# leodd/Lifted-Hybrid-Variational-Inference

Measured on AMD Instinct MI355X. Metric: lbp_sweeps_per_sec_10M_edge_hybrid_mrf, higher is better.
Workload: dtype f64

## Files before the change

### include/lhvi.h

```cpp
#ifndef LHVI_H
#define LHVI_H

#include <stddef.h>
#include <stdint.h>

#ifdef __cplusplus
extern "C" {
#endif

#define LHVI_ABI_VERSION 21
#define LHVI_MAX_ARITY 6

#define LHVI_OK 0
#define LHVI_E_ARG (-1)
#define LHVI_E_LAUNCH (-2)
#define LHVI_E_UNSUPPORTED (-3)
#define LHVI_E_NODEVICE (-4)
#define LHVI_E_NOT_PD (-5)

#define LHVI_POT_GENERIC 0
#define LHVI_POT_TABLE 1
#define LHVI_POT_GAUSSIAN 2
#define LHVI_POT_QUADRATIC 3
#define LHVI_POT_HYBRID_QUADRATIC 4
#define LHVI_POT_LINEAR_GAUSSIAN 5
#define LHVI_POT_X2 6
#define LHVI_POT_XY 7
#define LHVI_POT_MLN 8
#define LHVI_POT_MLN_HARD 9
#define LHVI_POT_IMAGE_NODE 10
#define LHVI_POT_IMAGE_EDGE 11

typedef struct lhvi_graph {
// ... 168 lines not shown
int lhvi_pbp_classify(const lhvi_graph_t* g, const lhvi_pots_t* pots, const lhvi_pbp_t* s, uint8_t* edge_class, void* stream);

int lhvi_pbp_uniq(const lhvi_graph_t* g, int32_t n, const double* particles, const int32_t* np, uint8_t* uniq, void* stream);
int lhvi_pbp_v2f(const lhvi_graph_t* g, const lhvi_pbp_t* s, const double* f2v, double* v2f, void* stream);
int lhvi_pbp_f2v(const lhvi_graph_t* g, const lhvi_pots_t* pots, const lhvi_pbp_t* s, const double* v2f, double* f2v, void* stream);
int lhvi_pbp_proposal(const lhvi_graph_t* g, const lhvi_pbp_t* s, const double* f2v, double* eta, double* q, void* stream);
int lhvi_pbp_proposal_partial(const lhvi_graph_t* g, const lhvi_pbp_t* s, const double* f2v, double* eta, double* ph, void* stream);
int lhvi_pbp_proposal_finish(const lhvi_graph_t* g, const lhvi_pbp_t* s, const double* ph, double* q, void* stream);
int lhvi_pbp_boundary_pack(const lhvi_graph_t* g, const lhvi_pbp_t* s, const double* f2v, const double* ph, int32_t nb,
                           const int32_t* bvars, double* send, void* stream);
int lhvi_pbp_boundary_reduce(int32_t n_items, const int32_t* width, const int32_t* src_ptr, const int64_t* src_off,
                             const int32_t* dst_ptr, const int64_t* dst_off, const double* in, double* out, void* stream);
int lhvi_pbp_init(const lhvi_graph_t* g, const lhvi_pbp_t* s, double* eta, double* q, double* f2v, double* v2f, void* stream);
int lhvi_pbp_resample(const lhvi_graph_t* g, const lhvi_pbp_t* s, const int64_t* var_gid, uint64_t seed, uint32_t iteration, double* particles_out, void* stream);
int lhvi_pbp_edge_points(const lhvi_graph_t* g, const lhvi_pots_t* pots, const lhvi_pbp_t* s, const double* v2f,
                         int32_t nq, const int32_t* qedge, int32_t npts, const double* x, double* out, void* stream);
int lhvi_pbp_resample_uniq(const lhvi_graph_t* g, const lhvi_pbp_t* s, const int64_t* var_gid, uint64_t seed, uint32_t iteration,
                           double* particles_out, uint8_t* uniq_out, void* stream);
int lhvi_pbp_belief_points(const lhvi_graph_t* g, const lhvi_pots_t* pots, const lhvi_pbp_t* s, const double* v2f,
                           int32_t nq, const int32_t* qvar, int32_t npts, const double* x, double* out, void* stream);
int lhvi_pbp_var_fused(const lhvi_graph_t* g, const lhvi_pbp_t* s, const double* f2v, double* v2f, double* eta, double* q,
                       const int64_t* var_gid, uint64_t seed, uint32_t iteration, double* particles_out, uint8_t* uniq_out,
                       const int32_t* desc, int32_t n16, int32_t n32_t32, int32_t n32_t64, void* stream);
int lhvi_pbp_quad(const lhvi_graph_t* g, const lhvi_pots_t* pots, const lhvi_pbp_t* s, const double* v2f, int64_t nq,
                  const int32_t* row_var, const int64_t* qptr, const int32_t* qedge, const double* qmult, const double* lo,
                  const double* hi, double epsabs, double epsrel, double* z, double* abserr, int32_t* status, void* stream);
int lhvi_pbp_map_brent(const lhvi_graph_t* g, const lhvi_pots_t* pots, const lhvi_pbp_t* s, const double* v2f, int64_t nq,
                       const int32_t* row_var, const int64_t* qptr, const int32_t* qedge, const double* qmult, double xtol,
                       int32_t maxfun, double* xout, double* fout, int32_t* nfev, void* stream);

int lhvi_pbp_halo_pack(const double* v2f, int32_t n, int32_t n_rows, const int32_t* row_edge, const int64_t* row_off,
                       const int32_t* row_width, const double* q, int32_t n_q, const int32_t* q_var, const int64_t* q_off,
                       double* out, void* stream);
int lhvi_pbp_halo_unpack(const double* in, int32_t n, int32_t n_rows, const int32_t* row_edge, const int64_t* row_off,
                         const int32_t* row_width, double* v2f, int32_t n_q, const int32_t* q_var, const int64_t* q_off,
                         double* q, void* stream);


typedef struct lhvi_vi {
    int32_t K;
    int32_t T;
    int32_t Dmax;
    int32_t quirks;
    const double* gh_x;
    const double* gh_w;
    const double* w;
// ... 262 lines not shown
```

### lifted-hybrid-variational-inference_amd/csrc/pbp.hip

```cpp
#include "common.hpp"
#include "potential.hpp"
#include "fastmath.hpp"
#include "cq.hpp"

namespace lhvi {

__device__ __forceinline__ double wave_sum(double v) { return dpp_wave_reduce(v, SumOp()); }
__device__ __forceinline__ double wave_max(double v) { return dpp_wave_reduce(v, MaxOp()); }
__device__ __forceinline__ int wave_sum_i(int v) {
#pragma unroll
    for (int off = 32; off > 0; off >>= 1) v += __shfl_xor(v, off);
    return v;
}

constexpr double PAD_LOG_TERM = -6.0e5;

__host__ __device__ __forceinline__ int var_first(const lhvi_pbp_t& s) { return s.var_hi > s.var_lo ? s.var_lo : 0; }
__host__ __device__ __forceinline__ int var_limit(const lhvi_graph_t& g, const lhvi_pbp_t& s) { return s.var_hi > s.var_lo ? s.var_hi : g.V; }

__device__ __forceinline__ double norm_pdf_std(double x, double mu, double sig) {
    const double u = (x - mu) / sig;
    return exp(-u * u * 0.5) / (2.506628274631 * sig);
}

// ... 2434 lines not shown
                uint64_t todo = dp & live;
                dp = 0;
                while (todo) {
                    const int k = __builtin_ctzll(todo);
                    const int klo = __builtin_amdgcn_readlane(xlo[h], k), khi = __builtin_amdgcn_readlane(xhi[h], k);
                    const uint64_t same = __ballot(xlo[h] == klo && xhi[h] == khi) & live;
                    dp |= same & (same - 1);
                    todo &= ~same;
                }
            }
            const int u = (lane < cn) && !((dp >> lane) & 1);
            if (lane < n) uniq[(int64_t)vv[h] * n + lane] = (uint8_t)u;
        }
    }
}

#ifndef LHVI_FUSED_WAVES
#define LHVI_FUSED_WAVES 4
#endif
constexpr int FUSED_CH = 8;
#ifndef LHVI_FUSED_NB
#define LHVI_FUSED_NB 2
#endif
template <int W, int PW, bool EP, bool R16>
__global__ void __launch_bounds__(BLOCK) __attribute__((amdgpu_waves_per_eu(LHVI_FUSED_WAVES, 8)))
pbp_var_fused_kernel(lhvi_graph_t g, lhvi_pbp_t s, const double* __restrict__ f2v, double* __restrict__ v2f, double* __restrict__ eta,
                     double* __restrict__ q, const int64_t* __restrict__ gid, uint64_t seed, uint32_t iteration,
                     double* __restrict__ out, uint8_t* __restrict__ uniq, const int32_t* __restrict__ list, int count) {
    __shared__ LogRec sh_log[LOG_TAB_N];
    load_log_table(sh_log);
    __syncthreads();
    constexpr int G = WAVE / W, SL = W / PW;
    const int lane = threadIdx.x & 63;
    const int64_t slot = ((int64_t)blockIdx.x * (BLOCK / WAVE) + (threadIdx.x >> 6)) * G + lane / W;
    const int j = lane % W;
    const bool on = slot < count;
    const int32_t* rec = list + (R16 ? 16 : 8) * (on ? slot : 0);
    int4 ra, rb;
    int2 rc = make_int2(0, 0);
    int e_rec = 0;
    if (R16) {
        const int4* r4 = reinterpret_cast<const int4*>(rec);
        ra = r4[0]; rb = r4[1]; rc = reinterpret_cast<const int2*>(rec)[4];
        e_rec = rec[10 + min(lane % W, 5)];
    } else {
        ra = make_int4(rec[0], rec[1], rec[2], rec[3]); rb = make_int4(rec[4], rec[5], rec[6], rec[7]);
    }
    const int v = on ? ra.x : 0;
    const int deg = on ? ra.y : 0, gb = ra.z, T = on ? ra.w : 0;
    const double dlo = __hiloint2double(rb.y, rb.x), dhi = __hiloint2double(rb.w, rb.z);
    const int n = s.n, S = s.n + s.T;
    const int np = on ? (R16 ? rc.x : s.np[v]) : 0;
    const bool valid = j < np;
    const int lo = on ? (R16 ? rc.y : g.var_ptr[v]) : 0;
    const bool lifted = g.edge_count != nullptr;
    const double q0 = on ? s.q[2 * v] : 0.0, q1 = on ? s.q[2 * v + 1] : 1.0;
    int maxdeg = deg;
#pragma unroll
    for (int off = 32; off >= W; off >>= 1) maxdeg = max(maxdeg, __shfl_xor(maxdeg, off));
    constexpr int CH = FUSED_CH;
    static_assert(W >= CH && CH % SL == 0, "lane j of a group holds edge j of the chunk");
    const int first_lane = lane / W * W;
    const int nch = (maxdeg + CH - 1) / CH;
    int my_e = 0, held = -1;
    auto hold_chunk = [&](int c) {
        if (c == held) return;
        held = c;
        if (R16 && c == 0) {
            my_e = j < deg ? (j < 6 ? e_rec : (j < CH ? g.var_edge[lo + j] : 0)) : 0;
            return;
        }
        my_e = (j < CH && c * CH + j < deg) ? g.var_edge[lo + c * CH + j] : 0;
    };
    {
        double total = 0.0;
        int ee[CH];
        double mm[CH];
        auto load_rows = [&](int c) {
            hold_chunk(c);
#pragma unroll
            for (int i = 0; i < CH; ++i) ee[i] = __shfl(my_e, first_lane + i);
#pragma unroll
            for (int i = 0; i < CH; ++i) mm[i] = f2v[(int64_t)ee[i] * S + (valid ? j : 0)];
        };
        for (int c = 0; c < nch; ++c) {
            load_rows(c);
#pragma unroll
            for (int i = 0; i < CH; ++i) {
                const double m = valid ? mm[i] : 0.0;
                if (c * CH + i < deg) total += lifted ? m * g.edge_count[ee[i]] : m;
            }
        }
        double logw = 0.0;
        bool uq = false;
        if (valid) {
            const int d = g.var_dom[v];
            const double sd = sqrt_pos(q1);
            logw = log_importance(g, s, v, d, s.particles[(int64_t)v * n + j], q0, rcp_newton(sd), log_pos(2.506628274631 * sd));
            uq = s.uniq[(int64_t)v * n + j] != 0;
        }
        auto group_sum = [&](double x) { return W == 16 ? dpp_move<0x15F>(dpp_row_reduce(x, SumOp())) : dpp_half_reduce(x, SumOp(), lane); };
        auto group_max = [&](double x) { return W == 16 ? dpp_row_reduce(x, MaxOp()) : dpp_half_reduce(x, MaxOp(), lane); };
        const uint64_t mine = (W == 16 ? 0xffffull : 0xffffffffull) << (lane / W * W);
        const double rcnt = rcp_newton(fmax((double)__builtin_popcountll(__ballot(uq) & mine), 1.0));
        for (int c = 0; c < nch; ++c) {
            if (nch > 1) load_rows(c);
#pragma unroll
            for (int i = 0; i < CH; ++i) {
                const int k = c * CH + i;
                if (k >= maxdeg) break;
                const bool live = k < deg;
                const double m = (live && valid) ? mm[i] : 0.0;
                const double res = (total - m) + logw;
                const double mean = group_sum(uq ? res : 0.0) * rcnt;
                double shift = mean;
                if (__ballot(uq && (res - mean > s.max_log_value))) {
                    const double mx = group_max(uq ? res : -__builtin_huge_val());
                    if (mx - mean > s.max_log_value) shift = mx - s.max_log_value;
                }
                if (live && valid) v2f[(int64_t)ee[i] * n + j] = res - shift;
            }
        }
    }
    double total = 0.0;
    if (lifted) for (int k = 0; k < deg; ++k) total += g.edge_count[g.var_edge[lo + k]];
    else total = (double)deg;
    const double min_sig = total * s.var_threshold;
    const int sub = j / PW, tl = j % PW;
    double ps[4] = {0.0, 0.0, 0.0, 0.0}, pm[4] = {0.0, 0.0, 0.0, 0.0};
    const int t0 = min(tl, max(T - 1, 0)), t1 = min(tl + PW, max(T - 1, 0));
    const double xg0 = g.dom_val[gb + t0], xg1 = g.dom_val[gb + t1];
    constexpr int NB = LHVI_FUSED_NB;
    for (int c = 0; c < nch; ++c) {
        hold_chunk(c);
#pragma unroll
        for (int p0 = 0; p0 < CH / SL; p0 += NB) {
            if (c * CH + p0 * SL >= maxdeg) break;
            int ee[NB];
            double b0[NB], b1[NB], g0[NB], g1[NB];
#pragma unroll
            for (int i = 0; i < NB; ++i) {
                const int kc = (p0 + i) * SL + sub;
                ee[i] = __shfl(my_e, first_lane + min(kc, CH - 1));
                if (kc >= CH || c * CH + kc >= deg) ee[i] = 0;
            }
#pragma unroll
            for (int i = 0; i < NB; ++i) {
                const double* msg = f2v + (int64_t)ee[i] * S + n;
                b0[i] = eta[2 * ee[i]]; b1[i] = eta[2 * ee[i] + 1];
                g0[i] = msg[t0]; g1[i] = msg[t1];
            }
#pragma unroll
            for (int i = 0; i < NB; ++i) {
                if (p0 + i >= CH / SL || c * CH + (p0 + i) * SL >= maxdeg) break;
                const int k = c * CH + (p0 + i) * SL + sub;
                const bool live = k < deg;
                const int e = ee[i];
                const double e0 = on ? b0[i] : 0.0, e1 = on ? b1[i] : 1.0;
                const bool use_cav = EP && !(q1 >= e1);
                double c0 = 0.0, c1 = 1.0;
                if (use_cav) gdiv(q0, q1, e0, e1, c0, c1);
                const double csd = sqrt(c1);
                double z = 0.0, a = 0.0, b = 0.0;
                if (on && tl < T) {
                    double w = exp(g0[i]);
                    if (use_cav) w = w * norm_pdf_std(xg0, c0, csd);
                    z += w; a += w * xg0; b += w * (xg0 * xg0);
                }
                if (on && tl + PW < T) {
                    double w = exp(g1[i]);
                    if (use_cav) w = w * norm_pdf_std(xg1, c0, csd);
                    z += w; a += w * xg1; b += w * (xg1 * xg1);
                }
                if (PW == 16) { z = dpp_row_reduce(z, SumOp()); a = dpp_row_reduce(a, SumOp()); b = dpp_row_reduce(b, SumOp()); }
                else { z = dpp_half_reduce(z, SumOp(), lane); a = dpp_half_reduce(a, SumOp(), lane); b = dpp_half_reduce(b, SumOp(), lane); }
                const double rz = rcp_newton(z);
                double mu = a * rz;
                double sig = b * rz - mu * mu;
                if (use_cav) { const double m0 = mu, m1 = sig; gdiv(m0, m1, c0, c1, mu, sig); }
                if (0.0 < sig && sig < __builtin_huge_val()) {
                    sig = fmax(sig, min_sig);
                    if (live && tl == 0) { eta[2 * e] = mu; eta[2 * e + 1] = sig; }
                } else {
                    mu = e0; sig = e1;
                }
                if (live) {
                    const double p = rcp_newton(sig);
                    const int slot4 = k & (WAVE / PW - 1);
                    const double cnt = lifted ? g.edge_count[e] : 1.0;
#pragma unroll
                    for (int r = 0; r < 4; ++r)
                        if (r == slot4) {
                            if (lifted) { ps[r] += p * cnt; pm[r] += p * mu * cnt; }
                            else { ps[r] += p; pm[r] += p * mu; }
                        }
                }
            }
        }
    }
    double fs, fm;
    if (PW == 16 && SL == 1) { fs = (ps[0] + ps[1]) + (ps[2] + ps[3]); fm = (pm[0] + pm[1]) + (pm[2] + pm[3]); }
    else if (PW == 16) {
        const double s01 = (sub == 0 ? ps[0] : ps[1]), s23 = (sub == 0 ? ps[2] : ps[3]);
        const double m01 = (sub == 0 ? pm[0] : pm[1]), m23 = (sub == 0 ? pm[2] : pm[3]);
        fs = (s01 + __shfl_xor(s01, 16)) + (s23 + __shfl_xor(s23, 16));
        fm = (m01 + __shfl_xor(m01, 16)) + (m23 + __shfl_xor(m23, 16));
    } else { fs = ps[0] + ps[1]; fm = pm[0] + pm[1]; }
    fs = 1.0 / fs;
    const double mu_new = fs * fm, var_new = fs;
    if (on && j == 0) { q[2 * v] = mu_new; q[2 * v + 1] = var_new; }
    const double mu_b = __shfl(mu_new, first_lane), sd_b = sqrt_pos(__shfl(var_new, first_lane));
    double x = 0.0;
    if (valid) {
        double zc, zs;
        philox_normal_pair(seed, gid ? (uint64_t)gid[v] : (uint64_t)v, (uint32_t)j, iteration, sh_log, zc, zs);
        x = fmin(fmax(fma(sd_b, zc, mu_b), dlo), dhi) + 0.0;
        out[(int64_t)v * n + j] = x;
    }
    int u = valid;
    for (int k = 0; k + 1 < W; ++k) {
        const double xk = __shfl(x, first_lane + k);
        if (k < j && k < np && xk == x) u = 0;
    }
    if (on && j < n) uniq[(int64_t)v * n + j] = (uint8_t)u;
}

static int validate_pbp(const lhvi_graph_t* g, const lhvi_pbp_t* s) {
    if (!g || !s) return LHVI_E_ARG;
    if (g->V < 0 || g->E < 0 || s->n <= 0 || s->T < 0) return LHVI_E_ARG;
    if (g->V > 0 && (!g->var_ptr || !g->var_edge || !g->var_value || !g->var_dom || !g->dom_cont || !g->dom_ptr ||
                     !s->particles || !s->np)) return LHVI_E_ARG;
    if (s->var_hi > s->var_lo ? (s->var_lo < 0 || s->var_hi > g->V) : (s->var_lo != 0 || s->var_hi != 0)) return LHVI_E_ARG;
    return LHVI_OK;
}

}

using namespace lhvi;

template <bool HALO>
static int launch_v2f(const lhvi_graph_t* g, const lhvi_pbp_t* s, const double* f2v, double* v2f, void* stream) {
    if (s->v2f_wide || s->v2f_narrow) {
        if (!s->v2f_wide || !s->v2f_narrow || s->n_v2f_wide < 0 || s->n_v2f_narrow < 0 || s->bslot || s->var_hi > s->var_lo) return LHVI_E_ARG;
        if (s->n_v2f_wide > 0)
            hipLaunchKernelGGL(pbp_v2f_kernel<HALO>, dim3(grid_for((int64_t)s->n_v2f_wide * WAVE)), dim3(BLOCK), 0, as_stream(stream), *g, *s, f2v, v2f);
// ... 383 lines not shown
    hipStream_t st = as_stream(stream);
    const bool ep = (s->flags & LHVI_PBP_EP) != 0;
#define LHVI_FUSED(W, PW, list, cnt)                                                                                                  \
    if ((cnt) > 0) {                                                                                                                  \
        const dim3 grid(grid_for(((int64_t)(cnt) + WAVE / (W) - 1) / (WAVE / (W)) * WAVE));                                          \
        if (ep && r16) hipLaunchKernelGGL((pbp_var_fused_kernel<W, PW, true, true>), grid, dim3(BLOCK), 0, st, *g, *s, f2v, v2f, eta, q, var_gid, \
                                   seed, iteration, particles_out, uniq_out, list, cnt);                                             \
        else if (ep) hipLaunchKernelGGL((pbp_var_fused_kernel<W, PW, true, false>), grid, dim3(BLOCK), 0, st, *g, *s, f2v, v2f, eta, q, var_gid, \
                                   seed, iteration, particles_out, uniq_out, list, cnt);                                             \
        else if (r16) hipLaunchKernelGGL((pbp_var_fused_kernel<W, PW, false, true>), grid, dim3(BLOCK), 0, st, *g, *s, f2v, v2f, eta, q, var_gid,   \
                                seed, iteration, particles_out, uniq_out, list, cnt);                                                \
        else hipLaunchKernelGGL((pbp_var_fused_kernel<W, PW, false, false>), grid, dim3(BLOCK), 0, st, *g, *s, f2v, v2f, eta, q, var_gid,   \
                                seed, iteration, particles_out, uniq_out, list, cnt);                                                \
    }
    const bool r16 = (s->flags & LHVI_PBP_FUSED_RECORDS16) != 0;
    const int64_t rw = r16 ? 16 : 8;
    LHVI_FUSED(16, 16, desc, n16)
    LHVI_FUSED(32, 16, desc + rw * (int64_t)n16, n32_t32)
    LHVI_FUSED(32, 32, desc + rw * ((int64_t)n16 + n32_t32), n32_t64)
#undef LHVI_FUSED
    return check_launch();
}

int lhvi_pbp_quad(const lhvi_graph_t* g, const lhvi_pots_t* pots, const lhvi_pbp_t* s, const double* v2f, int64_t nq,
                  const int32_t* row_var, const int64_t* qptr, const int32_t* qedge, const double* qmult, const double* lo,
                  const double* hi, double epsabs, double epsrel, double* z, double* abserr, int32_t* status, void* stream) {
    if (int rc = validate_pbp(g, s)) return rc;
    if (!pots || !v2f || nq < 0 || !(epsabs >= 0.0) || !(epsrel >= 0.0)) return LHVI_E_ARG;
    if (nq == 0) return LHVI_OK;
    if (!row_var || !lo || !hi || !z) return LHVI_E_ARG;
    if (qptr && (!qedge || !qmult)) return LHVI_E_ARG;
    QueryRows rows{row_var, qptr, qedge, qmult};
    hipLaunchKernelGGL(pbp_quad_kernel, dim3(grid_for(nq)), dim3(BLOCK), 0, as_stream(stream), *g, *pots, *s, v2f, nq, rows, row_var,
                       lo, hi, epsabs, epsrel, z, abserr, status);
    return check_launch();
}

}
```

### lifted-hybrid-variational-inference_amd/lhvi/_abi.py

```python
from __future__ import annotations

import ctypes as C
import os

import numpy as np

_HERE = os.path.dirname(os.path.abspath(__file__))
LIB_PATH = os.environ.get('LHVI_LIB') or os.path.join(os.path.dirname(_HERE), 'csrc', 'liblhvi.so')

c_i32p = C.c_void_p
c_f64p = C.c_void_p


class LhviError(RuntimeError):
    pass


class GraphStruct(C.Structure):
    _fields_ = [
        ('V', C.c_int32), ('F', C.c_int32), ('E', C.c_int32), ('nnz', C.c_int32),
        ('fac_ptr', C.c_void_p), ('edge_var', C.c_void_p), ('edge_fac', C.c_void_p), ('edge_canon', C.c_void_p),
        ('var_ptr', C.c_void_p), ('var_edge', C.c_void_p), ('edge_count', C.c_void_p), ('fac_pot', C.c_void_p),
        ('var_value', C.c_void_p), ('var_dom', C.c_void_p), ('var_mult', C.c_void_p), ('fac_mult', C.c_void_p),
        ('D', C.c_int32),
# ... 52 lines not shown
               [(n, C.c_double) for n in ('lr', 'b1', 'b2', 'eps', 'var_min')] + [('t', C.c_int32)]


PBP_EP = 1
PBP_EPBP_DISCRETE = 2
PBP_SKIP_TERMS = 16
PBP_NO_GRID = 128
PBP_LEAVE_ROOM = 256
PBP_BOUNDARY_TOTALS = 2048
PBP_CQ = 512
PBP_NO_UNIQ = 4096
PBP_V2F_RECORDS = 8192
PBP_WIDE_PAIRS = 16384
PBP_SHARE_CUS = 32768
PBP_POW2_GROUPS = 65536
PBP_FUSED_RECORDS16 = 131072
PBP_F2V_HEAVY = 262144
PBP_F2V_SMALL = 524288
PBP_F2V_PAIR = 1048576
PBP_F2V_FAST = 2097152
PBP_F2V_CQ = 4194304
PBP_F2V_GENERIC = 8388608
PBP_F2V_ALL = PBP_F2V_HEAVY | PBP_F2V_SMALL | PBP_F2V_PAIR | PBP_F2V_FAST | PBP_F2V_CQ | PBP_F2V_GENERIC
ABI_VERSION = 21
PBP_DESC_BYTES = 128
COLOR_HASH, COLOR_SORT = 0, 1
HUB_DEGREE = 64
VI_GROUP_SLOTS, VI_GROUP_COMP, VI_TINY_NODES, VI_TINY_K, VI_TINY_PAR = 24, 48, 32, 2, 3072

class MwsStruct(C.Structure):
    _fields_ = [('T', C.c_int32), ('max_flips', C.c_int32), ('epsilon', C.c_double), ('noise_std', C.c_double),
                ('seed', C.c_uint64), ('try_id', C.c_void_p), ('disc', C.c_void_p), ('n_disc', C.c_int32),
                ('num', C.c_void_p), ('n_num', C.c_int32), ('fac_class', C.c_void_p), ('x', C.c_void_p), ('best_x', C.c_void_p),
                ('cur_score', C.c_void_p), ('best_score', C.c_void_p), ('status', C.c_void_p), ('err_flip', C.c_void_p),
                ('rec_score', C.c_void_p), ('rec_zero', C.c_void_p), ('rec_ticks', C.c_void_p)] + \
               [(n, C.c_void_p) for n in ('rp_init', 'rp_clause', 'rp_walk', 'rp_walk_k', 'rp_noise', 'rp_post', 'out_score',
                                          'out_unsat', 'out_winner', 'out_accept', 'out_val')]


class ExactStruct(C.Structure):
    _fields_ = [('Nd', C.c_int32), ('Nc', C.c_int32), ('M', C.c_int64), ('dstates', C.c_void_p), ('dstride', C.c_void_p),
                ('n_quad', C.c_int32), ('quad_ptr', C.c_void_p), ('quad_desc', C.c_void_p), ('quad_par', C.c_void_p),
                ('n_tab', C.c_int32), ('tab_ptr', C.c_void_p), ('tab_desc', C.c_void_p), ('tab_par', C.c_void_p)]


class GibbsStruct(C.Structure):
    _fields_ = [('ex', ExactStruct), ('dstate_off', C.c_void_p), ('vt_ptr', C.c_void_p), ('vt_fac', C.c_void_p),
# ... 58 lines not shown
    'lhvi_pbp_var_sum': (C.c_int, [_G, _S, _vp, _vp, _vp]),
    'lhvi_pbp_domain_grid': (C.c_int, [_G, _S, _vp, _vp]),
    'lhvi_pbp_refine_grid': (C.c_int, [_G, _S, _vp, _vp, _vp, _vp, _vp]),
    'lhvi_debug_exp': (C.c_int, [_vp, _vp, _i64, _vp]),
    'lhvi_debug_log': (C.c_int, [_vp, _vp, _i64, C.c_int32, _vp]),
    'lhvi_debug_exp_acc': (C.c_int, [_vp, _vp, _vp, _i64, _vp]),
    'lhvi_debug_exp_acc_floor': (C.c_int, [_vp, _vp, _vp, _i64, _vp]),
    'lhvi_pbp_v2f': (C.c_int, [_G, _S, _vp, _vp, _vp]),
    'lhvi_pbp_f2v': (C.c_int, [_G, _P, _S, _vp, _vp, _vp]),
    'lhvi_pbp_proposal': (C.c_int, [_G, _S, _vp, _vp, _vp, _vp]),
    'lhvi_pbp_proposal_partial': (C.c_int, [_G, _S, _vp, _vp, _vp, _vp]),
    'lhvi_pbp_proposal_finish': (C.c_int, [_G, _S, _vp, _vp, _vp]),
    'lhvi_pbp_boundary_pack': (C.c_int, [_G, _S, _vp, _vp, _i32, _vp, _vp, _vp]),
    'lhvi_pbp_boundary_reduce': (C.c_int, [_i32, _vp, _vp, _vp, _vp, _vp, _vp, _vp, _vp]),
    'lhvi_pbp_halo_pack': (C.c_int, [_vp, _i32, _i32, _vp, _vp, _vp, _vp, _i32, _vp, _vp, _vp, _vp]),
    'lhvi_pbp_halo_unpack': (C.c_int, [_vp, _i32, _i32, _vp, _vp, _vp, _vp, _i32, _vp, _vp, _vp, _vp]),
    'lhvi_pbp_init': (C.c_int, [_G, _S, _vp, _vp, _vp, _vp, _vp]),
    'lhvi_pbp_resample': (C.c_int, [_G, _S, _vp, _u64, _u32, _vp, _vp]),
    'lhvi_pbp_edge_points': (C.c_int, [_G, _P, _S, _vp, _i32, _vp, _i32, _vp, _vp, _vp]),
    'lhvi_pbp_resample_uniq': (C.c_int, [_G, _S, _vp, _u64, _u32, _vp, _vp, _vp]),
    'lhvi_pbp_belief_points': (C.c_int, [_G, _P, _S, _vp, _i32, _vp, _i32, _vp, _vp, _vp]),
    'lhvi_pbp_map_brent': (C.c_int, [_G, _P, _S, _vp, _i64, _vp, _vp, _vp, _vp, _f64, _i32, _vp, _vp, _vp, _vp]),
    'lhvi_pbp_var_fused': (C.c_int, [_G, _S, _vp, _vp, _vp, _vp, _vp, _u64, _u32, _vp, _vp, _vp, _i32, _i32, _i32, _vp]),
    'lhvi_pbp_quad': (C.c_int, [_G, _P, _S, _vp, _i64, _vp, _vp, _vp, _vp, _vp, _vp, _f64, _f64, _vp, _vp, _vp, _vp]),
    'lhvi_vi_workspace_bytes': (_sz, [_G, _VI]),
    'lhvi_vi_grad': (C.c_int, [_G, _P, _VI, _vp, _vp, _vp, _vp, _vp, _sz, _vp]),
    'lhvi_vi_adam_run': (C.c_int, [_G, _P, _VI, C.POINTER(ViOptStruct), _i32, _vp, _vp, _sz, _vp]),
    'lhvi_adam_step': (C.c_int, [_vp, _vp, _vp, _vp, _i64, _i32, _f64, _f64, _f64, _f64, _i32, _f64, _vp]),
    'lhvi_softmax_rows': (C.c_int, [_vp, _vp, _i64, _i32, _i32, _vp]),
    'lhvi_vi_map_bfgs': (C.c_int, [_G, _VI, _i64, _vp, _f64, _i32, _vp, _vp, _vp, _vp, _vp]),
    'lhvi_color_workspace_bytes': (_sz, [_G]),
    'lhvi_color_refine_factors': (C.c_int, [_G, _vp, _vp, _vp, _vp, _vp, _vp, _sz, _i32, _vp]),
    'lhvi_color_refine_rvs': (C.c_int, [_G, _vp, _vp, _vp, _vp, _vp, _sz, _i32, _vp]),
    'lhvi_color_first_members': (C.c_int, [_vp, _i32, _i32, _vp, _vp]),
    'lhvi_color_segment_sums': (C.c_int, [_vp, _vp, _i32, _vp, _vp]),
    'lhvi_mws_init': (C.c_int, [_G, _P, C.POINTER(MwsStruct), _vp]),
    'lhvi_mws_flips': (C.c_int, [_G, _P, C.POINTER(MwsStruct), _i32, _i32, _vp]),
    'lhvi_lbfgsb_host': (C.c_int, [_i32, _vp, LBFGSB_FUN, _vp, _vp, _vp, _vp, _vp]),
    'lhvi_wall_clock_khz': (C.c_int, [_vp]),
    'lhvi_exact_lds_bytes': (_sz, [_i32, _i32, _i32]),
    'lhvi_exact_configs': (C.c_int, [C.POINTER(ExactStruct), _i64, _i64, _i32, _vp, _vp, _vp, _vp, _vp, _vp]),
    'lhvi_exact_normalize': (C.c_int, [_i64, _vp, _vp, _vp, _vp, _vp]),
    'lhvi_exact_marginals': (C.c_int, [C.POINTER(ExactStruct), _i32, _vp, _vp, _vp]),
    'lhvi_exact_mix_prepare': (C.c_int, [_i32, _i64, _vp, _vp, _vp, _vp, _vp]),
    'lhvi_exact_mixture': (C.c_int, [_i32, _i64, _vp, _i32, _vp, _vp, _vp]),
    'lhvi_exact_map_polish': (C.c_int, [_i32, _i64, _vp, _i32, _vp, _vp, _vp, _vp, _i32, _vp, _vp]),
# ... 227 lines not shown
```

### lifted-hybrid-variational-inference_amd/lhvi/pbp.py

```python
from __future__ import annotations

import os
from math import e, log, sqrt

import numpy as np

from . import _abi
from .flat import flatten

_F2V_LONG = _abi.PBP_F2V_HEAVY | _abi.PBP_F2V_SMALL
_F2V_SHORT = _abi.PBP_F2V_PAIR | _abi.PBP_F2V_FAST | _abi.PBP_F2V_CQ | _abi.PBP_F2V_GENERIC
F2V_SCHEDULES = {
    'one': (('main', _abi.PBP_F2V_ALL, 0, False),),
    'timed': (('main', _F2V_LONG, 0, True), ('main', _F2V_SHORT, 0, False)),
    'overlap': (('side', _F2V_SHORT, 0, False), ('main', _F2V_LONG, _abi.PBP_SHARE_CUS, True)),
}


class _ParticleSweep:
    var_threshold = 3
    max_log_value = 700
    _epbp_discrete = True
    verbose = False
    listed_proposal = True
    dynamic_f2v = True
    paired_light = True
    cq_routing = True
    small_f2v = True
    long_grid_min_edges = 1 << 16
    listed_resample = True
    sliced_proposal = True
    prop_slice = 64
    packed_v2f = True
    overlap_f2v = True
    overlap_min_heavy = 1 << 16
    fused_var_kernel = True
    fused_max_particles = 32
    exact_queries = False
    map_mode = 'fminbound'

    def _setup(self, graph_like, flat=None, edge_key=None, sides='vf', edge_skip=None, owned=None):
        flat = flat if flat is not None else flatten(graph_like, require_device_potentials=True)
        self.flat = flat
        self.dg = dg = _abi.DeviceGraph(flat)
        torch = _abi.require_gpu()
        n = self.n
        sizes = np.diff(flat.dom_ptr)
        cont = flat.dom_cont.astype(bool)
        self.T = int(sizes[cont].max()) if cont.any() else 0
        nst = flat.var_nstates
        if (flat.var_hidden & ~flat.var_cont & (nst > n)).any():
            raise _abi.LhviError('a discrete variable has more states than particle slots n=%d' % n)
        if (flat.var_hidden & flat.var_cont & (np.diff(flat.var_ptr) == 0)).any():
            raise ZeroDivisionError('a hidden continuous variable has no incident factor: its proposal is an empty product')
        self.np_host = np.where(flat.var_hidden, np.where(flat.var_cont, n, nst), 0).astype(np.int32)
        host_lists = {'np_dev': self.np_host}
        S = n + self.T
        self.f2v = dg.zeros(flat.E, S)
        self.v2f = dg.zeros(flat.E, n)
        self.eta = dg.zeros(flat.E, 2)
# ... 47 lines not shown
            pd = np.concatenate([sl, np.delete(pd, hubs, axis=0)])
            host_lists['prop_hub'], self.n_prop_hub = ph, int(hubs.size)
            self.prop_partial = dg.zeros(owner.size, 2)
        host_lists['prop_desc'] = np.ascontiguousarray(pd) if pv.size else None
        self.n_prop_desc = int(pd.shape[0])
        hidden_v = np.flatnonzero(flat.var_hidden)
        if owned is not None:
            hidden_v = hidden_v[hidden_v < owned]
        narrow = self.np_host[hidden_v] <= 4
        self.v2f_lists = None
        hub = ~narrow & (np.diff(flat.var_ptr)[hidden_v] > 64) & (self.np_host[hidden_v] <= 64)
        mid16 = ~narrow & ~hub & (self.np_host[hidden_v] <= 16)
        mid32 = ~narrow & ~hub & ~mid16 & (self.np_host[hidden_v] <= 32)
        if self.packed_v2f and hidden_v.size and (narrow.any() or hub.any() or mid16.any() or mid32.any()):
            wide = ~narrow & ~hub & ~mid16 & ~mid32
            parts = (('wide', wide), ('narrow', narrow), ('hub', hub), ('mid16', mid16), ('mid32', mid32))
            for name, m in parts:
                host_lists['v2f_' + name] = hidden_v[m].astype(np.int32) if m.any() else np.zeros(1, dtype=np.int32)
            if os.environ.get('LHVI_PBP_V2F_REC', '1') != '0':
                host_lists['v2f_wide'] = self._v2f_records(flat, hidden_v[wide])
        self._fused = None
        pT = sizes[pdom] if pv.size else np.zeros(0, dtype=np.int64)
        fused_max = int(os.environ.get('LHVI_PBP_FUSED_MAX', self.fused_max_particles))
        fz = (pdeg <= min(64, self.prop_slice)) & (pT <= 64) & (n <= min(32, fused_max)) if pv.size else np.zeros(0, dtype=bool)
        if (self.fused_var_kernel and os.environ.get('LHVI_PBP_FUSED', '1') != '0') and owned is None and self.sampler == 'device' and self.listed_proposal and self.listed_resample \
                and 'v2f_wide' in host_lists and fz.any():
            k16 = fz & (n <= 16) & (pT <= 32)
            k32a = fz & ~k16 & (pT <= 32)
            k32b = fz & ~k16 & ~k32a
            wide_rec = os.environ.get('LHVI_PBP_FUSED_REC16', '1') != '0'
            fd = np.zeros((pv.size, 16 if wide_rec else 8), dtype=np.int32)
            fd[:, 0], fd[:, 1], fd[:, 2], fd[:, 3] = pv, pdeg, flat.dom_ptr[pdom], pT
            fd[:, 4:6] = np.ascontiguousarray(flat.dom_lo[pdom], dtype=np.float64).view(np.int32).reshape(-1, 2)
            fd[:, 6:8] = np.ascontiguousarray(flat.dom_hi[pdom], dtype=np.float64).view(np.int32).reshape(-1, 2)
            if wide_rec:
                fd[:, 8], fd[:, 9] = self.np_host[pv], flat.var_ptr[pv]
                for k in range(6):
                    has = pdeg > k
                    fd[has, 10 + k] = flat.var_edge[pbase[has] + k]
                self.flags |= _abi.PBP_FUSED_RECORDS16
            host_lists['fused_desc'] = np.ascontiguousarray(np.concatenate([fd[k16], fd[k32a], fd[k32b]]))
            fused_var = np.zeros(flat.V, dtype=bool)
            fused_var[pv[fz]] = True
            keep = ~fused_var[pd[:, 0]]
            host_lists['prop_desc_rest'] = np.ascontiguousarray(pd[keep]) if keep.any() else np.zeros((1, 8), dtype=np.int32)
            rkeep = ~fused_var[rr[:, 0]]
            host_lists['resample_rest'] = np.ascontiguousarray(rr[rkeep]) if rkeep.any() else np.zeros((1, 8), dtype=np.int32)
            rest_parts = []
            if 'v2f_wide' in host_lists:
                for name, m in parts:
                    vs = hidden_v[m]
                    vs = vs[~fused_var[vs]]
                    host_lists['v2f_rest_' + name] = (self._v2f_records(flat, vs) if name == 'wide' and os.environ.get('LHVI_PBP_V2F_REC', '1') != '0' else
                                                      vs.astype(np.int32) if vs.size else np.zeros(1, dtype=np.int32))
                    rest_parts.append((name, int(vs.size)))
            self._fused = dict(counts=(int(k16.sum()), int(k32a.sum()), int(k32b.sum())), n_prop_rest=int(keep.sum()),
                               n_resample_rest=int(rkeep.sum()), rest_parts=rest_parts)
        dev_lists = _abi.upload(host_lists)
        for name in ('np_dev', 'resample_vars', '_static_idx', 'prop_desc'):
            setattr(self, name, dev_lists[name])
        if self._fused is not None:
            F = self._fused
            F['desc'], F['prop_desc_rest'], F['resample_rest'] = dev_lists['fused_desc'], dev_lists['prop_desc_rest'], dev_lists['resample_rest']
            F['v2f_rest'] = tuple(x for name, cnt in F['rest_parts'] for x in (dev_lists['v2f_rest_' + name], cnt)) if F['rest_parts'] else None
        if 'prop_hub' in dev_lists:
            self.prop_hub = dev_lists['prop_hub']
        if 'v2f_wide' in dev_lists:
            self.v2f_lists = tuple(x for name, m in parts for x in (dev_lists['v2f_' + name], int(m.sum())))
            if os.environ.get('LHVI_PBP_V2F_REC', '1') != '0':
                self.flags |= _abi.PBP_V2F_RECORDS
        pad = torch.zeros(1, dtype=torch.int32, device=dg.device)
        self.cq_edges = pad[:0]
        self.part_counts = {'heavy': 0, 'light': 0, 'fast': 0, 'generic': 0, 'cq': 0, 'pair': 0, 'small16': 0, 'small32': 0}
        self.generic_pts_log2 = 6
        self.fast_desc = self.heavy_desc = self.light_desc = self.pair_desc = self.small16_desc = self.small32_desc = None
        self.n_heavy = self.n_light = self.n_pair = self.n_small16 = self.n_small32 = self.n_heavy_class = 0
        self.cq_terms = self.heavy_terms = self.heavy_grid_terms = 0
        self._has_f_side = 'f' in sides
        if not self._has_f_side:
            self.fast_edges = self.generic_edges = pad[:0]
            self._fast_list = self._generic_list = pad
            return
        cls = torch.zeros(max(flat.E, 1), dtype=torch.uint8, device=dg.device)
        _abi.check(_abi.lib().lhvi_pbp_classify(dg.g, dg.p, self._struct(), _abi.ptr(cls), _abi.stream_ptr()))
        cls = cls[:flat.E]
        if edge_skip is not None:
# ... 211 lines not shown
        elif callable(self.sampler):
            self._install(self.sampler(k, self.flat, self.q_dev.cpu().numpy()))
        else:
            self._install(self._host_draw())
        _abi.check(l.lhvi_pbp_uniq(self.dg.g, self.n, _abi.ptr(self.particles), _abi.ptr(self.np_dev),
                                   _abi.ptr(self.uniq), st))
        self._views, self._batched = {}, {}

    def _run_sweeps(self, iteration):
        l, st, g, p = _abi.lib(), _abi.stream_ptr(), self.dg.g, self.dg.p
        _abi.check(l.lhvi_pbp_init(g, self._struct(), _abi.ptr(self.eta), _abi.ptr(self.q_dev), _abi.ptr(self.f2v),
                                   _abi.ptr(self.v2f), st))
        self._generate_sample()
        for i in range(iteration):
            self.sweep(last=(i == iteration - 1))
        self._views, self._batched = {}, {}

    def sweep(self, last=False, f2v_events=None):
        l, st, g, p = _abi.lib(), _abi.stream_ptr(), self.dg.g, self.dg.p
        if not last and getattr(self, '_fused', None) is not None and self._static_rows and self.sampler == 'device':
            F = self._fused
            s = self._struct()
            n16, n32a, n32b = F['counts']
            _abi.check(l.lhvi_pbp_var_fused(g, s, _abi.ptr(self.f2v), _abi.ptr(self.v2f), _abi.ptr(self.eta), _abi.ptr(self.q_dev),
                                            _abi.ptr(getattr(self, 'var_gid', None)), int(self.seed), int(self._draws),
                                            _abi.ptr(self.old_particles), _abi.ptr(self.uniq), _abi.ptr(F['desc']), n16, n32a, n32b, st))
            w, nw, nr, nn, hb, nh, m16, c16, m32, c32 = F['v2f_rest']
            s.v2f_wide, s.n_v2f_wide, s.v2f_narrow, s.n_v2f_narrow = _abi.ptr(w), nw, _abi.ptr(nr), nn
            s.v2f_hub, s.n_v2f_hub = _abi.ptr(hb), nh
            s.v2f_mid16, s.n_v2f_mid16, s.v2f_mid32, s.n_v2f_mid32 = _abi.ptr(m16), c16, _abi.ptr(m32), c32
            _abi.check(l.lhvi_pbp_v2f(g, s, _abi.ptr(self.f2v), _abi.ptr(self.v2f), st))
            s.prop_desc, s.n_prop_desc = _abi.ptr(F['prop_desc_rest']), int(F['n_prop_rest'])
            _abi.check(l.lhvi_pbp_proposal(g, s, _abi.ptr(self.f2v), _abi.ptr(self.eta), _abi.ptr(self.q_dev), st))
            self._generate_sample(rest_only=True)
            self._launch_f2v(self._struct(), f2v_events)
            return
        _abi.check(l.lhvi_pbp_v2f(g, self._struct(), _abi.ptr(self.f2v), _abi.ptr(self.v2f), st))
        if not last:
            _abi.check(l.lhvi_pbp_proposal(g, self._struct(), _abi.ptr(self.f2v), _abi.ptr(self.eta),
                                           _abi.ptr(self.q_dev), st))
            self._generate_sample()
            self._launch_f2v(self._struct(), f2v_events)

    def _f2v_schedule(self, timed=False):
        want = os.environ.get('LHVI_PBP_OVERLAP')
        if (self.overlap_f2v or want == '1') and want != '0' and self.n_heavy >= self.overlap_min_heavy:
            return 'overlap'
        return 'timed' if timed else 'one'

# ... 838 lines not shown
```

Before: 68.37.

## Extend fused variable kernel to 64-particle variables with one wavefront each

Adds a W=64 instantiation of the fused v2f/proposal/resample kernel and a new entry point, so variables with 33 to 64 particles also take the fused path instead of separate v2f, proposal and resample launches. The 64-wide form uses whole-wave reductions, a single accumulator slot, and an LDS hash to detect duplicate particles, replacing the quadratic shuffle loop. It also prefetches the first chunk's proposal inputs and defers the log-table fill to cut early latency. The risk is higher register and LDS pressure, and the RNG lane mapping changes for these variables.

```diff
diff --git a/include/lhvi.h b/include/lhvi.h
--- a/include/lhvi.h
+++ b/include/lhvi.h
@@ -8,7 +8,7 @@
 extern "C" {
 #endif
 
-#define LHVI_ABI_VERSION 21
+#define LHVI_ABI_VERSION 22
 #define LHVI_MAX_ARITY 6
 
 #define LHVI_OK 0
@@ -223,6 +223,9 @@
 int lhvi_pbp_var_fused(const lhvi_graph_t* g, const lhvi_pbp_t* s, const double* f2v, double* v2f, double* eta, double* q,
                        const int64_t* var_gid, uint64_t seed, uint32_t iteration, double* particles_out, uint8_t* uniq_out,
                        const int32_t* desc, int32_t n16, int32_t n32_t32, int32_t n32_t64, void* stream);
+int lhvi_pbp_var_fused64(const lhvi_graph_t* g, const lhvi_pbp_t* s, const double* f2v, double* v2f, double* eta, double* q,
+                         const int64_t* var_gid, uint64_t seed, uint32_t iteration, double* particles_out, uint8_t* uniq_out,
+                         const int32_t* desc, int32_t n64_t32, int32_t n64_t64, void* stream);
 int lhvi_pbp_quad(const lhvi_graph_t* g, const lhvi_pots_t* pots, const lhvi_pbp_t* s, const double* v2f, int64_t nq,
                   const int32_t* row_var, const int64_t* qptr, const int32_t* qedge, const double* qmult, const double* lo,
                   const double* hi, double epsabs, double epsrel, double* z, double* abserr, int32_t* status, void* stream);
diff --git a/lifted-hybrid-variational-inference_amd/csrc/pbp.hip b/lifted-hybrid-variational-inference_amd/csrc/pbp.hip
--- a/lifted-hybrid-variational-inference_amd/csrc/pbp.hip
+++ b/lifted-hybrid-variational-inference_amd/csrc/pbp.hip
@@ -2480,17 +2480,42 @@
 #ifndef LHVI_FUSED_NB
 #define LHVI_FUSED_NB 2
 #endif
+#ifndef LHVI_FUSED64_WAVES
+#define LHVI_FUSED64_WAVES 8
+#endif
+#ifndef LHVI_FUSED64_CH
+#define LHVI_FUSED64_CH 4
+#endif
+#ifndef LHVI_FUSED64_PRE
+#define LHVI_FUSED64_PRE 1
+#endif
+#ifndef LHVI_FUSED64_EARLY
+#define LHVI_FUSED64_EARLY 1
+#endif
+#ifndef LHVI_FUSED64_LATE_TABLE
+#define LHVI_FUSED64_LATE_TABLE 1
+#endif
+constexpr int FUSED_CH64 = LHVI_FUSED64_CH;
+constexpr int FUSED64_HASH_BITS = 12;
 template <int W, int PW, bool EP, bool R16>
-__global__ void __launch_bounds__(BLOCK) __attribute__((amdgpu_waves_per_eu(LHVI_FUSED_WAVES, 8)))
+__global__ void __launch_bounds__(BLOCK) __attribute__((amdgpu_waves_per_eu(W == 64 ? (PW == 32 || EP ? LHVI_FUSED_WAVES : LHVI_FUSED64_WAVES) : LHVI_FUSED_WAVES, 8)))
 pbp_var_fused_kernel(lhvi_graph_t g, lhvi_pbp_t s, const double* __restrict__ f2v, double* __restrict__ v2f, double* __restrict__ eta,
                      double* __restrict__ q, const int64_t* __restrict__ gid, uint64_t seed, uint32_t iteration,
                      double* __restrict__ out, uint8_t* __restrict__ uniq, const int32_t* __restrict__ list, int count) {
     __shared__ LogRec sh_log[LOG_TAB_N];
-    load_log_table(sh_log);
-    __syncthreads();
+    __shared__ uint8_t sh_owner[W == 64 ? (BLOCK / WAVE) << FUSED64_HASH_BITS : 1];
+    constexpr bool LATE_TABLE = W == 64 && LHVI_FUSED64_LATE_TABLE != 0;
+    double tab_inv = 0.0, tab_log = 0.0;
+    if constexpr (LATE_TABLE) {
+        if (threadIdx.x < LOG_TAB_N) { tab_inv = LOG_TAB[2 * threadIdx.x]; tab_log = LOG_TAB[2 * threadIdx.x + 1]; }
+    } else {
+        load_log_table(sh_log);
+        __syncthreads();
+    }
     constexpr int G = WAVE / W, SL = W / PW;
     const int lane = threadIdx.x & 63;
-    const int64_t slot = ((int64_t)blockIdx.x * (BLOCK / WAVE) + (threadIdx.x >> 6)) * G + lane / W;
+    const int wave = W == 64 ? __builtin_amdgcn_readfirstlane(threadIdx.x >> 6) : (int)(threadIdx.x >> 6);
+    const int64_t slot = ((int64_t)blockIdx.x * (BLOCK / WAVE) + wave) * G + lane / W;
     const int j = lane % W;
     const bool on = slot < count;
     const int32_t* rec = list + (R16 ? 16 : 8) * (on ? slot : 0);
@@ -2516,8 +2541,9 @@
     int maxdeg = deg;
 #pragma unroll
     for (int off = 32; off >= W; off >>= 1) maxdeg = max(maxdeg, __shfl_xor(maxdeg, off));
-    constexpr int CH = FUSED_CH;
+    constexpr int CH = W == 64 ? FUSED_CH64 : FUSED_CH;
     static_assert(W >= CH && CH % SL == 0, "lane j of a group holds edge j of the chunk");
+    static_assert(W < 64 || R16, "the one-variable-per-wavefront form reads sixteen-word records");
     const int first_lane = lane / W * W;
     const int nch = (maxdeg + CH - 1) / CH;
     int my_e = 0, held = -1;
@@ -2530,6 +2556,18 @@
         }
         my_e = (j < CH && c * CH + j < deg) ? g.var_edge[lo + c * CH + j] : 0;
     };
+    constexpr bool PRE = W == 64 && LHVI_FUSED64_PRE != 0;
+    int pre_e = 0;
+    double pre_b0 = 0.0, pre_b1 = 1.0, pre_g0 = 0.0, pre_g1 = 0.0;
+    auto preload = [&]() {
+        const int psub = j / PW, ptl = j % PW;
+        const int pt0 = min(ptl, max(T - 1, 0)), pt1 = min(ptl + PW, max(T - 1, 0));
+        pre_e = __shfl(my_e, first_lane + min(psub, CH - 1));
+        if (psub >= CH || psub >= deg) pre_e = 0;
+        const double* msg = f2v + (int64_t)pre_e * S + n;
+        pre_b0 = eta[2 * pre_e]; pre_b1 = eta[2 * pre_e + 1];
+        pre_g0 = msg[pt0]; pre_g1 = msg[pt1];
+    };
     {
         double total = 0.0;
         int ee[CH];
@@ -2541,25 +2579,41 @@
 #pragma unroll
             for (int i = 0; i < CH; ++i) mm[i] = f2v[(int64_t)ee[i] * S + (valid ? j : 0)];
         };
+        constexpr bool EARLY = W == 64 && LHVI_FUSED64_EARLY != 0;
+        double logw = 0.0, early_x = 0.0;
+        bool uq = false;
+        auto importance = [&](double xp) {
+            const int d = g.var_dom[v];
+            const double sd = sqrt_pos(q1);
+            return log_importance(g, s, v, d, xp, q0, rcp_newton(sd), log_pos(2.506628274631 * sd));
+        };
+        if (EARLY && valid) {
+            early_x = s.particles[(int64_t)v * n + j];
+            uq = s.uniq[(int64_t)v * n + j] != 0;
+        }
         for (int c = 0; c < nch; ++c) {
             load_rows(c);
+            if (PRE && c == 0) preload();
+            if (EARLY && c == 0 && valid) logw = importance(early_x);
 #pragma unroll
             for (int i = 0; i < CH; ++i) {
                 const double m = valid ? mm[i] : 0.0;
                 if (c * CH + i < deg) total += lifted ? m * g.edge_count[ee[i]] : m;
             }
         }
-        double logw = 0.0;
-        bool uq = false;
-        if (valid) {
-            const int d = g.var_dom[v];
-            const double sd = sqrt_pos(q1);
-            logw = log_importance(g, s, v, d, s.particles[(int64_t)v * n + j], q0, rcp_newton(sd), log_pos(2.506628274631 * sd));
+        if (!EARLY && valid) {
+            logw = importance(s.particles[(int64_t)v * n + j]);
             uq = s.uniq[(int64_t)v * n + j] != 0;
         }
-        auto group_sum = [&](double x) { return W == 16 ? dpp_move<0x15F>(dpp_row_reduce(x, SumOp())) : dpp_half_reduce(x, SumOp(), lane); };
-        auto group_max = [&](double x) { return W == 16 ? dpp_row_reduce(x, MaxOp()) : dpp_half_reduce(x, MaxOp(), lane); };
-        const uint64_t mine = (W == 16 ? 0xffffull : 0xffffffffull) << (lane / W * W);
+        auto group_sum = [&](double x) {
+            if constexpr (W == 64) return wave_sum(x);
+            else return W == 16 ? dpp_move<0x15F>(dpp_row_reduce(x, SumOp())) : dpp_half_reduce(x, SumOp(), lane);
+        };
+        auto group_max = [&](double x) {
+            if constexpr (W == 64) return wave_max(x);
+            else return W == 16 ? dpp_row_reduce(x, MaxOp()) : dpp_half_reduce(x, MaxOp(), lane);
+        };
+        const uint64_t mine = W == 64 ? ~0ull : (W == 16 ? 0xffffull : 0xffffffffull) << (lane / W * W);
         const double rcnt = rcp_newton(fmax((double)__builtin_popcountll(__ballot(uq) & mine), 1.0));
         for (int c = 0; c < nch; ++c) {
             if (nch > 1) load_rows(c);
@@ -2588,7 +2642,7 @@
     double ps[4] = {0.0, 0.0, 0.0, 0.0}, pm[4] = {0.0, 0.0, 0.0, 0.0};
     const int t0 = min(tl, max(T - 1, 0)), t1 = min(tl + PW, max(T - 1, 0));
     const double xg0 = g.dom_val[gb + t0], xg1 = g.dom_val[gb + t1];
-    constexpr int NB = LHVI_FUSED_NB;
+    constexpr int NB = W == 64 ? (LHVI_FUSED_NB < CH / SL ? LHVI_FUSED_NB : CH / SL) : LHVI_FUSED_NB;
     for (int c = 0; c < nch; ++c) {
         hold_chunk(c);
 #pragma unroll
@@ -2604,6 +2658,10 @@
             }
 #pragma unroll
             for (int i = 0; i < NB; ++i) {
+                if (PRE && p0 + i == 0 && c == 0) {
+                    b0[i] = pre_b0; b1[i] = pre_b1; g0[i] = pre_g0; g1[i] = pre_g1;
+                    continue;
+                }
                 const double* msg = f2v + (int64_t)ee[i] * S + n;
                 b0[i] = eta[2 * ee[i]]; b1[i] = eta[2 * ee[i] + 1];
                 g0[i] = msg[t0]; g1[i] = msg[t1];
@@ -2646,18 +2704,27 @@
                     const double p = rcp_newton(sig);
                     const int slot4 = k & (WAVE / PW - 1);
                     const double cnt = lifted ? g.edge_count[e] : 1.0;
-#pragma unroll
-                    for (int r = 0; r < 4; ++r)
-                        if (r == slot4) {
-                            if (lifted) { ps[r] += p * cnt; pm[r] += p * mu * cnt; }
-                            else { ps[r] += p; pm[r] += p * mu; }
-                        }
+                    if constexpr (W == 64) {
+                        if (lifted) { ps[0] += p * cnt; pm[0] += p * mu * cnt; }
+                        else { ps[0] += p; pm[0] += p * mu; }
+                    } else {
+#pragma unroll
+                        for (int r = 0; r < 4; ++r)
+                            if (r == slot4) {
+                                if (lifted) { ps[r] += p * cnt; pm[r] += p * mu * cnt; }
+                                else { ps[r] += p; pm[r] += p * mu; }
+                            }
+                    }
                 }
             }
         }
     }
     double fs, fm;
-    if (PW == 16 && SL == 1) { fs = (ps[0] + ps[1]) + (ps[2] + ps[3]); fm = (pm[0] + pm[1]) + (pm[2] + pm[3]); }
+    if constexpr (W == 64) {
+        fs = ps[0]; fm = pm[0];
+#pragma unroll
+        for (int off = PW; off < 64; off <<= 1) { fs += __shfl_xor(fs, off); fm += __shfl_xor(fm, off); }
+    } else if (PW == 16 && SL == 1) { fs = (ps[0] + ps[1]) + (ps[2] + ps[3]); fm = (pm[0] + pm[1]) + (pm[2] + pm[3]); }
     else if (PW == 16) {
         const double s01 = (sub == 0 ? ps[0] : ps[1]), s23 = (sub == 0 ? ps[2] : ps[3]);
         const double m01 = (sub == 0 ? pm[0] : pm[1]), m23 = (sub == 0 ? pm[2] : pm[3]);
@@ -2667,18 +2734,43 @@
     fs = 1.0 / fs;
     const double mu_new = fs * fm, var_new = fs;
     if (on && j == 0) { q[2 * v] = mu_new; q[2 * v + 1] = var_new; }
+    if constexpr (LATE_TABLE) {
+        static_assert(LOG_TAB_N <= BLOCK, "one table entry per thread");
+        if (threadIdx.x < LOG_TAB_N) { sh_log[threadIdx.x].inv_c = tab_inv; sh_log[threadIdx.x].log_c = tab_log; }
+        __syncthreads();
+    }
     const double mu_b = __shfl(mu_new, first_lane), sd_b = sqrt_pos(__shfl(var_new, first_lane));
     double x = 0.0;
     if (valid) {
         double zc, zs;
-        philox_normal_pair(seed, gid ? (uint64_t)gid[v] : (uint64_t)v, (uint32_t)j, iteration, sh_log, zc, zs);
+        philox_normal_pair(seed, gid ? (uint64_t)gid[v] : (uint64_t)v, (uint32_t)(W == 64 ? j & 31 : j), iteration, sh_log, zc, zs);
+        if (W == 64 && (j & 32)) zc = zs;
         x = fmin(fmax(fma(sd_b, zc, mu_b), dlo), dhi) + 0.0;
         out[(int64_t)v * n + j] = x;
     }
     int u = valid;
-    for (int k = 0; k + 1 < W; ++k) {
-        const double xk = __shfl(x, first_lane + k);
-        if (k < j && k < np && xk == x) u = 0;
+    if constexpr (W == 64) {
+        volatile uint8_t* owner = sh_owner + ((threadIdx.x >> 6) << FUSED64_HASH_BITS);
+        const int xlo = __double2loint(x), xhi = __double2hiint(x);
+        const uint32_t h = (((uint32_t)xlo * 0x9E3779B1u) ^ ((uint32_t)xhi * 0x85EBCA6Bu)) >> (32 - FUSED64_HASH_BITS);
+        if (valid) owner[h] = (uint8_t)lane;
+        LHVI_WAVE_SYNC();
+        const bool suspect = valid && owner[h] != (uint8_t)lane;
+        const uint64_t live = __ballot(valid);
+        uint64_t todo = __ballot(suspect), dp = 0;
+        while (todo) {
+            const int k = __builtin_ctzll(todo);
+            const int klo = __builtin_amdgcn_readlane(xlo, k), khi = __builtin_amdgcn_readlane(xhi, k);
+            const uint64_t same = __ballot(xlo == klo && xhi == khi) & live;
+            dp |= same & (same - 1);
+            todo &= ~same;
+        }
+        u = valid && !((dp >> lane) & 1);
+    } else {
+        for (int k = 0; k + 1 < W; ++k) {
+            const double xk = __shfl(x, first_lane + k);
+            if (k < j && k < np && xk == x) u = 0;
+        }
     }
     if (on && j < n) uniq[(int64_t)v * n + j] = (uint8_t)u;
 }
@@ -3108,6 +3200,30 @@
     return check_launch();
 }
 
+int lhvi_pbp_var_fused64(const lhvi_graph_t* g, const lhvi_pbp_t* s, const double* f2v, double* v2f, double* eta, double* q,
+                         const int64_t* var_gid, uint64_t seed, uint32_t iteration, double* particles_out, uint8_t* uniq_out,
+                         const int32_t* desc, int32_t n64_t32, int32_t n64_t64, void* stream) {
+    if (int rc = validate_pbp(g, s)) return rc;
+    if (!f2v || !v2f || !eta || !q || !particles_out || !uniq_out || !s->uniq || !s->q || !g->dom_lo || !g->dom_hi || !g->dom_val) return LHVI_E_ARG;
+    if (n64_t32 < 0 || n64_t64 < 0 || s->n <= 32 || s->n > 64 || s->bslot || s->var_hi > s->var_lo || particles_out == s->particles) return LHVI_E_ARG;
+    if ((int64_t)n64_t32 + n64_t64 == 0) return LHVI_OK;
+    if (!desc) return LHVI_E_ARG;
+    hipStream_t st = as_stream(stream);
+    const bool ep = (s->flags & LHVI_PBP_EP) != 0;
+#define LHVI_FUSED64(PW, list, cnt)                                                                                                   \
+    if ((cnt) > 0) {                                                                                                                  \
+        const dim3 grid(grid_for((int64_t)(cnt) * WAVE));                                                                             \
+        if (ep) hipLaunchKernelGGL((pbp_var_fused_kernel<64, PW, true, true>), grid, dim3(BLOCK), 0, st, *g, *s, f2v, v2f, eta, q, var_gid, \
+                                   seed, iteration, particles_out, uniq_out, list, cnt);                                             \
+        else hipLaunchKernelGGL((pbp_var_fused_kernel<64, PW, false, true>), grid, dim3(BLOCK), 0, st, *g, *s, f2v, v2f, eta, q, var_gid,   \
+                                seed, iteration, particles_out, uniq_out, list, cnt);                                                \
+    }
+    LHVI_FUSED64(16, desc, n64_t32)
+    LHVI_FUSED64(32, desc + 16 * (int64_t)n64_t32, n64_t64)
+#undef LHVI_FUSED64
+    return check_launch();
+}
+
 int lhvi_pbp_quad(const lhvi_graph_t* g, const lhvi_pots_t* pots, const lhvi_pbp_t* s, const double* v2f, int64_t nq,
                   const int32_t* row_var, const int64_t* qptr, const int32_t* qedge, const double* qmult, const double* lo,
                   const double* hi, double epsabs, double epsrel, double* z, double* abserr, int32_t* status, void* stream) {
diff --git a/lifted-hybrid-variational-inference_amd/lhvi/_abi.py b/lifted-hybrid-variational-inference_amd/lhvi/_abi.py
--- a/lifted-hybrid-variational-inference_amd/lhvi/_abi.py
+++ b/lifted-hybrid-variational-inference_amd/lhvi/_abi.py
@@ -98,7 +98,7 @@
 PBP_F2V_CQ = 4194304
 PBP_F2V_GENERIC = 8388608
 PBP_F2V_ALL = PBP_F2V_HEAVY | PBP_F2V_SMALL | PBP_F2V_PAIR | PBP_F2V_FAST | PBP_F2V_CQ | PBP_F2V_GENERIC
-ABI_VERSION = 21
+ABI_VERSION = 22
 PBP_DESC_BYTES = 128
 COLOR_HASH, COLOR_SORT = 0, 1
 HUB_DEGREE = 64
@@ -203,6 +203,7 @@
     'lhvi_pbp_belief_points': (C.c_int, [_G, _P, _S, _vp, _i32, _vp, _i32, _vp, _vp, _vp]),
     'lhvi_pbp_map_brent': (C.c_int, [_G, _P, _S, _vp, _i64, _vp, _vp, _vp, _vp, _f64, _i32, _vp, _vp, _vp, _vp]),
     'lhvi_pbp_var_fused': (C.c_int, [_G, _S, _vp, _vp, _vp, _vp, _vp, _u64, _u32, _vp, _vp, _vp, _i32, _i32, _i32, _vp]),
+    'lhvi_pbp_var_fused64': (C.c_int, [_G, _S, _vp, _vp, _vp, _vp, _vp, _u64, _u32, _vp, _vp, _vp, _i32, _i32, _vp]),
     'lhvi_pbp_quad': (C.c_int, [_G, _P, _S, _vp, _i64, _vp, _vp, _vp, _vp, _vp, _vp, _f64, _f64, _vp, _vp, _vp, _vp]),
     'lhvi_vi_workspace_bytes': (_sz, [_G, _VI]),
     'lhvi_vi_grad': (C.c_int, [_G, _P, _VI, _vp, _vp, _vp, _vp, _vp, _sz, _vp]),
diff --git a/lifted-hybrid-variational-inference_amd/lhvi/pbp.py b/lifted-hybrid-variational-inference_amd/lhvi/pbp.py
--- a/lifted-hybrid-variational-inference_amd/lhvi/pbp.py
+++ b/lifted-hybrid-variational-inference_amd/lhvi/pbp.py
@@ -35,7 +35,7 @@
     overlap_f2v = True
     overlap_min_heavy = 1 << 16
     fused_var_kernel = True
-    fused_max_particles = 32
+    fused_max_particles = 64
     exact_queries = False
     map_mode = 'fminbound'
 
@@ -129,24 +129,38 @@
         self._fused = None
         pT = sizes[pdom] if pv.size else np.zeros(0, dtype=np.int64)
         fused_max = int(os.environ.get('LHVI_PBP_FUSED_MAX', self.fused_max_particles))
-        fz = (pdeg <= min(64, self.prop_slice)) & (pT <= 64) & (n <= min(32, fused_max)) if pv.size else np.zeros(0, dtype=bool)
+        fz = (pdeg <= min(64, self.prop_slice)) & (pT <= 64) & (n <= min(64, fused_max)) if pv.size else np.zeros(0, dtype=bool)
         if (self.fused_var_kernel and os.environ.get('LHVI_PBP_FUSED', '1') != '0') and owned is None and self.sampler == 'device' and self.listed_proposal and self.listed_resample \
                 and 'v2f_wide' in host_lists and fz.any():
             k16 = fz & (n <= 16) & (pT <= 32)
-            k32a = fz & ~k16 & (pT <= 32)
-            k32b = fz & ~k16 & ~k32a
+            k32a = fz & (n <= 32) & ~k16 & (pT <= 32)
+            k32b = fz & (n <= 32) & ~k16 & ~k32a
+            k64a = fz & (n > 32) & (pT <= 32)
+            k64b = fz & (n > 32) & ~k64a
             wide_rec = os.environ.get('LHVI_PBP_FUSED_REC16', '1') != '0'
             fd = np.zeros((pv.size, 16 if wide_rec else 8), dtype=np.int32)
             fd[:, 0], fd[:, 1], fd[:, 2], fd[:, 3] = pv, pdeg, flat.dom_ptr[pdom], pT
             fd[:, 4:6] = np.ascontiguousarray(flat.dom_lo[pdom], dtype=np.float64).view(np.int32).reshape(-1, 2)
             fd[:, 6:8] = np.ascontiguousarray(flat.dom_hi[pdom], dtype=np.float64).view(np.int32).reshape(-1, 2)
+            def sixteen(rec8):
+                rec = np.zeros((pv.size, 16), dtype=np.int32)
+                rec[:, :8] = rec8
+                rec[:, 8], rec[:, 9] = self.np_host[pv], flat.var_ptr[pv]
+                for k in range(6):
+                    has = pdeg > k
+                    rec[has, 10 + k] = flat.var_edge[pbase[has] + k]
+                return rec
             if wide_rec:
                 fd[:, 8], fd[:, 9] = self.np_host[pv], flat.var_ptr[pv]
                 for k in range(6):
                     has = pdeg > k
                     fd[has, 10 + k] = flat.var_edge[pbase[has] + k]
                 self.flags |= _abi.PBP_FUSED_RECORDS16
-            host_lists['fused_desc'] = np.ascontiguousarray(np.concatenate([fd[k16], fd[k32a], fd[k32b]]))
+            small = np.concatenate([fd[k16], fd[k32a], fd[k32b]])
+            host_lists['fused_desc'] = np.ascontiguousarray(small) if small.size else np.zeros((1, fd.shape[1]), dtype=np.int32)
+            if k64a.any() or k64b.any():
+                fd64 = fd if wide_rec else sixteen(fd[:, :8])
+                host_lists['fused64_desc'] = np.ascontiguousarray(np.concatenate([fd64[k64a], fd64[k64b]]))
             fused_var = np.zeros(flat.V, dtype=bool)
             fused_var[pv[fz]] = True
             keep = ~fused_var[pd[:, 0]]
@@ -161,14 +175,15 @@
                     host_lists['v2f_rest_' + name] = (self._v2f_records(flat, vs) if name == 'wide' and os.environ.get('LHVI_PBP_V2F_REC', '1') != '0' else
                                                       vs.astype(np.int32) if vs.size else np.zeros(1, dtype=np.int32))
                     rest_parts.append((name, int(vs.size)))
-            self._fused = dict(counts=(int(k16.sum()), int(k32a.sum()), int(k32b.sum())), n_prop_rest=int(keep.sum()),
-                               n_resample_rest=int(rkeep.sum()), rest_parts=rest_parts)
+            self._fused = dict(counts=(int(k16.sum()), int(k32a.sum()), int(k32b.sum())), counts64=(int(k64a.sum()), int(k64b.sum())),
+                               n_prop_rest=int(keep.sum()), n_resample_rest=int(rkeep.sum()), rest_parts=rest_parts)
         dev_lists = _abi.upload(host_lists)
         for name in ('np_dev', 'resample_vars', '_static_idx', 'prop_desc'):
             setattr(self, name, dev_lists[name])
         if self._fused is not None:
             F = self._fused
             F['desc'], F['prop_desc_rest'], F['resample_rest'] = dev_lists['fused_desc'], dev_lists['prop_desc_rest'], dev_lists['resample_rest']
+            F['desc64'] = dev_lists.get('fused64_desc')
             F['v2f_rest'] = tuple(x for name, cnt in F['rest_parts'] for x in (dev_lists['v2f_rest_' + name], cnt)) if F['rest_parts'] else None
         if 'prop_hub' in dev_lists:
             self.prop_hub = dev_lists['prop_hub']
@@ -426,9 +441,15 @@
             F = self._fused
             s = self._struct()
             n16, n32a, n32b = F['counts']
-            _abi.check(l.lhvi_pbp_var_fused(g, s, _abi.ptr(self.f2v), _abi.ptr(self.v2f), _abi.ptr(self.eta), _abi.ptr(self.q_dev),
-                                            _abi.ptr(getattr(self, 'var_gid', None)), int(self.seed), int(self._draws),
-                                            _abi.ptr(self.old_particles), _abi.ptr(self.uniq), _abi.ptr(F['desc']), n16, n32a, n32b, st))
+            if n16 + n32a + n32b:
+                _abi.check(l.lhvi_pbp_var_fused(g, s, _abi.ptr(self.f2v), _abi.ptr(self.v2f), _abi.ptr(self.eta), _abi.ptr(self.q_dev),
+                                                _abi.ptr(getattr(self, 'var_gid', None)), int(self.seed), int(self._draws),
+                                                _abi.ptr(self.old_particles), _abi.ptr(self.uniq), _abi.ptr(F['desc']), n16, n32a, n32b, st))
+            if F['desc64'] is not None:
+                n64a, n64b = F['counts64']
+                _abi.check(l.lhvi_pbp_var_fused64(g, s, _abi.ptr(self.f2v), _abi.ptr(self.v2f), _abi.ptr(self.eta), _abi.ptr(self.q_dev),
+                                                  _abi.ptr(getattr(self, 'var_gid', None)), int(self.seed), int(self._draws),
+                                                  _abi.ptr(self.old_particles), _abi.ptr(self.uniq), _abi.ptr(F['desc64']), n64a, n64b, st))
             w, nw, nr, nn, hb, nh, m16, c16, m32, c32 = F['v2f_rest']
             s.v2f_wide, s.n_v2f_wide, s.v2f_narrow, s.n_v2f_narrow = _abi.ptr(w), nw, _abi.ptr(nr), nn
             s.v2f_hub, s.n_v2f_hub = _abi.ptr(hb), nh
```

New measurement: 70.69, median of 6. 1.03x the previous value.
